# xultaeculcis/climate-super-resolution

Hardware: AMD Instinct MI355X
Metric: HR MPix/s per training step (4x SR, 64->256 tiles) (higher is better)
Workload: dtype bf16; 1 GPU; config 3: full ESRGAN GAN step (pl_gan.py:63-97: G pass = G fwd + D(hr), D(sr) + VGG19 perceptual + L1 + G bwd + AdamW_G; D pass = G fwd + D(hr), D(sr) + D bwd + AdamW_D; OneCycleLR x2); generator=ESRGAN nf64 nb11 gc16 x4, discriminator=RFBESRGANDiscriminator, global_batch=32, per_gpu_batch=32, lr_tile=64, hr_tile=256, parallelism=dp1, hip_graph=True, ddp_overlap=False, mode=gan

## Files before the change

### climate-super-resolution_amd/csrc/common.h

```cpp
#pragma once
#include <hip/hip_runtime.h>
#include <stdint.h>

#include "climsr_hip.h"

typedef __bf16 bf16x8 __attribute__((ext_vector_type(8)));
typedef __bf16 bf16x2 __attribute__((ext_vector_type(2)));
typedef short s16x4 __attribute__((ext_vector_type(4)));
typedef float f32x4 __attribute__((ext_vector_type(4)));

namespace climsr {

void set_error(const char* fmt, ...);
int check_launch(const char* what);
int device_cus();
int lds_opt_in(const void* fn, int bytes);

__device__ __forceinline__ uint16_t f2bf(float f) {
  __bf16 b = (__bf16)f;
  return __builtin_bit_cast(uint16_t, b);
}
__device__ __forceinline__ float bf2f(uint16_t u) { return __uint_as_float(((uint32_t)u) << 16); }

__device__ __forceinline__ float act_apply(float v, int act, float slope) {
// ... 15 lines not shown
constexpr uint32_t BUF_OOB = 0x80000000u;
__device__ __forceinline__ __amdgpu_buffer_rsrc_t buf_rsrc(const void* base, uint32_t bytes) {
  return __builtin_amdgcn_make_buffer_rsrc(const_cast<void*>(base), (short)0, (int)bytes, 0x00020000);
}
__device__ __forceinline__ uint4 buf_load16(__amdgpu_buffer_rsrc_t r, uint32_t off) {
  const auto v = __builtin_amdgcn_raw_buffer_load_b128(r, off, 0, 0);
  return make_uint4(v[0], v[1], v[2], v[3]);
}

__device__ __forceinline__ void lds_barrier() {
  __builtin_amdgcn_fence(__ATOMIC_RELEASE, "workgroup", "local");
  __builtin_amdgcn_s_barrier();
  __builtin_amdgcn_fence(__ATOMIC_ACQUIRE, "workgroup", "local");
}

static inline int ceil_div(long a, long b) { return (int)((a + b - 1) / b); }
static inline int round_up(int a, int b) { return (a + b - 1) / b * b; }

}
```

### climate-super-resolution_amd/csrc/conv.hip

```cpp
#include <atomic>
#include <mutex>
#include <stdarg.h>
#include <stdio.h>
#include <stdlib.h>

#include "common.h"
#include "conv_ep.h"
#include "conv_route.h"

namespace climsr {

static thread_local char g_err[512] = "";

void set_error(const char* fmt, ...) {
  va_list ap;
  va_start(ap, fmt);
  vsnprintf(g_err, sizeof(g_err), fmt, ap);
  va_end(ap);
}

int check_launch(const char* what) {
  hipError_t e = hipGetLastError();
  if (e != hipSuccess) {
    set_error("%s: %s", what, hipGetErrorString(e));
// ... 354 lines not shown
    r->geo = 2;
    if (r->pg.nvx <= 2 * 64 * r->nw) r->pv = 2;
  } else if (r->nw * r->mw == 16 && d->ks == 3 && d->cc == 64 && r->pg.kcpad == 9 * 64 && r->pg.ccp == 80 && r->pg.tpw == TW + 2 &&
             r->pg.tph == 18) {
    r->geo = 1;
  }
  r->tiles_y = ceil_div(d->out_h, r->nw * r->mw);
  return true;
}

static void pick_generic(const ClimsrConvDesc* d, bool bias, const ClimsrEpilogue* ep, bool bz, FwdRoute* r) {
  const FwdGeom& g = r->g;
  const bool r1 = ep->res1 != nullptr, r2 = ep->res2 != nullptr, aux = ep->aux != nullptr, bwd = ep->act == 3 || ep->act == 4;
  const bool al8 = (d->out_c & 7) == 0 && ((d->out_cstride | d->out_coff) & 7) == 0;
  const bool r1al8 = ((ep->res1_cstride | ep->res1_coff) & 7) == 0;
  const int plain = plain_ep(d, bias, ep);
  r->family = FAM_FWD; r->mw = g.mw; r->nt = g.nt;
  r->parts = bz && d->up == -2 && plain == 8 && dgrad_s2_shape(d, bias, ep);
  if (g.mw == 4) {
    const int nrx = ceil_div(g.tph * g.tpw * (d->cc / 8), 256), nrw = ceil_div(g.nt * 16 * (g.kcpad / 8), 256);
    r->nt = 4;
    if (g.nchunk > 1 && nrx <= 6 && nrw <= 9) {
      r->pfx = 6; r->pfw = 9;
      const bool v8 = al8 && r1al8 && (!r2 || ((ep->res2_cstride | ep->res2_coff) & 7) == 0) &&
                      (!aux || ((ep->aux_cstride | ep->aux_coff) & 7) == 0) && !ep->down2 && ep->act == 0 && r1;
      if (v8 && bias && ep->res_f32 == 0 && ep->out_mode == 0 && !aux) r->ep = 1;
      else if (v8 && !bias && (ep->res_f32 & 1) && (!r2 || (ep->res_f32 & 2)) && ep->out_mode == 1) r->ep = 2;
      else if (!bias && r1 && bwd && ep->res_f32 == 0 && !r2 && !aux && !ep->down2 && ep->out_mode == 0 && al8 && r1al8) r->ep = 4;
      else if (plain == 8) r->ep = bz ? 10 : ep->bn_part ? 9 : 8;
      else r->ep = plain;
      r->parts |= (r->ep == 9 || r->ep == 10) && d->out_c % 64 == 0 && d->out_c >= 128 && d->stride == 1 && d->up == 1 && d->ks == 3;
    } else if (g.nchunk > 1 && nrx <= 18 && nrw <= 9) {
      r->pfx = 18; r->pfw = 9; r->ep = plain == 8 ? 8 : 0;
    } else {
      r->ep = plain;
    }
    const bool base = d->cc == 32 && d->ks == 3 && g.kcpad == 9 * 32;
    if (r->pfx != 18 && base && d->stride == 1 && g.tpw == TW + 2 && g.ccp == 48 && d->up == 1 && d->in_c % 32 == 0 &&
        g.nchunk * 32 == d->in_c && (long)d->n * d->in_h * d->in_w * d->in_cstride * 2 < (1L << 31) &&
        (long)r->ncob * r->nt * 16 * g.kpk * 2 < (1L << 31))
      r->geo = 1;
    if (r->pfx == 18 && base && d->stride == 2 && g.tpw == 2 * TW + 1 && g.ccp == 40) r->geo = 2;
  }
  if (r->geo == 1) {
    const bool fits = (r->ep == 9 || r->ep == 10) ? d->out_h % DMA_TH == 0 : (d->out_h % DMA_TH == 0 || d->out_h >= 3 * DMA_TH);
    if (r->ep != 1 && r->ep != 2 && !ep->down2 && fits) {
      r->family = FAM_DMA;
      r->tiles_y = ceil_div(d->out_h, DMA_TH);
      r->xgrp = conv_xcd_group(r->ncob, (long)64 * g.kpk * 2);
      return;
    }
    r->xgrp = conv_xcd_group(r->ncob, (long)r->nt * 16 * g.kpk * 2);
  }
  const size_t lds_ep = (size_t)4 * r->mw * 16 * (r->nt * 16 + 4) * 4;
  r->lds = lds_ep > g.lds_total ? lds_ep : g.lds_total;
}

static int fwd_pick(const ClimsrConvDesc* d, bool bias, const ClimsrEpilogue* ep, FwdRoute* r) {
  *r = FwdRoute{};
  const bool cc4 = d->cc == 4 && d->in_c == 4;
  const bool bz = ep->bn_part && ep->bn_z, r1 = ep->res1 != nullptr, r2 = ep->res2 != nullptr, aux = ep->aux != nullptr;
// ... 52 lines not shown
}

static int fwd_route(const ClimsrConvDesc* d, bool bias, const ClimsrEpilogue* ep, FwdRoute* r) {
  if (!d || !ep) {
    set_error("conv2d_fwd: null argument");
    return CLIMSR_EINVAL;
  }
  const bool cc4 = d->cc == 4 && d->in_c == 4;
  if ((d->in_c % 8 && !cc4) || d->in_cstride % 8 || d->in_coff % 8 || (d->cc % 8 && !cc4) || d->cc <= 0 ||
      (d->up != 1 && d->up != 2 && d->up != -2) ||
      (d->stride != 1 && d->stride != 2) || d->ks < 1 || d->n <= 0 || d->out_c <= 0 || d->in_coff + d->in_c > d->in_cstride) {
    set_error("conv2d_fwd: unsupported geometry (in_c=%d cs=%d coff=%d cc=%d up=%d stride=%d ks=%d)", d->in_c, d->in_cstride,
              d->in_coff, d->cc, d->up, d->stride, d->ks);
    return CLIMSR_EINVAL;
  }
  if (ep->down2 && (ep->res2 || ep->res_f32 || bias || ep->act == 1 || ep->act == 2 || (ep->res1 && ep->act < 3) ||
                    (d->out_h & 1) || (d->out_w & 1))) {
    set_error("conv2d_fwd: down2 epilogue: no bias / forward activation / residual (act 3/4 mask only), even output size");
    return CLIMSR_EINVAL;
  }
  if (ep->act < 0 || ep->act > 4 || ((ep->act == 3 || ep->act == 4) && !ep->res1)) {
    set_error("conv2d_fwd: act %d invalid (3/4 need res1 = the activation output)", ep->act);
    return CLIMSR_EINVAL;
  }
  const int pick = fwd_pick(d, bias, ep, r);
  if (ep->ch_part && !(pick == PICK_OK && r->family == FAM_WR && (r->ep == 3 || r->ep == 4))) {
    set_error("conv2d_fwd: per-tile channel sums only from the 64 -> 64 3x3 register-resident conv "
              "(climsr_conv2d_fwd_ch_parts)");
    return CLIMSR_EINVAL;
  }
  if (ep->aux && ((ep->aux_cstride | ep->aux_coff) & 3)) {
    set_error("conv2d_fwd: aux channel stride/offset must be multiples of 4");
    return CLIMSR_EINVAL;
  }
  {
    const long opx = (long)d->n * d->out_h * d->out_w;
    const long r1b = ep->res1 ? opx * ep->res1_cstride * ((ep->res_f32 & 1) ? 4 : 2) : 0;
    const long r2b = ep->res2 ? opx * ep->res2_cstride * ((ep->res_f32 & 2) ? 4 : 2) : 0;
    const long yb = opx * d->out_cstride * (ep->out_mode == 0 ? 2 : 4);
    if (r1b >= (1L << 32) - 64 || r2b >= (1L << 32) - 64 || yb >= (1L << 32) - 64) {
      set_error("conv2d_fwd: output / residual operand of %ld B exceeds 32-bit buffer addressing (split the batch)",
// ... 130 lines not shown
```

### climate-super-resolution_amd/csrc/conv_dma.hip

```cpp
#include <algorithm>
#include <type_traits>

#include "conv_ep.h"

constexpr int DMA_TPW = TW + 2, DMA_XROW = DMA_TPW * 64;
constexpr int DMA_XU = (DMA_TH + 2) * DMA_TPW * 4;
constexpr int DMA_XI = (DMA_XU + 63) / 64;
constexpr int DMA_WI = 64 * 36 / 64;
constexpr int DMA_XB = DMA_XI * 1024, DMA_WB = DMA_WI * 1024, DMA_BUF = DMA_XB + DMA_WB;
constexpr int DMA_EPP = 64 + 4;
constexpr size_t DMA_LDS = std::max((size_t)2 * DMA_BUF, (size_t)8 * 64 * DMA_EPP * 4);
static_assert(DMA_LDS <= 160 * 1024, "LDS-DMA conv: two chunk buffers");


constexpr uint32_t ST_OOB = 0xFFFFFFC0u;
typedef unsigned int v4u32 __attribute__((ext_vector_type(4)));
template <int EP>
struct DmaEp {
  static constexpr bool F32 = EP == 2 || EP == 7;
  static constexpr int NSTORE = 4 * (F32 ? 2 : 1) + (EP == 2 ? 4 : 0);
};
template <int EP>
__device__ __forceinline__ void dma_store_half(const FwdArgs& a, const float* eb, int ehp, int lane, int nimg, int oyw, int ox0, int co0) {
  static_assert(EP == 1 || EP == 2 || EP == 3 || EP == 6 || EP == 7 || EP == 8, "persistent epilogues");
// ... 46 lines not shown
    if constexpr (EP == 2) __builtin_amdgcn_raw_buffer_store_b128(__builtin_bit_cast(v4u32, pack8_bf16(v, a.aux_scale)), rax, aoff[j], 0, 0);
  }
}

#ifndef CLIMSR_DMA_SPREAD
#define CLIMSR_DMA_SPREAD 1
#endif
#ifndef CLIMSR_DMA_DIAG
#define CLIMSR_DMA_DIAG 0
#endif

template <int EP, bool RF>
__global__ __launch_bounds__(512, 1) void conv_fwd_dma_kernel(FwdArgs a) {
  extern __shared__ __attribute__((aligned(16))) char smem[];
  constexpr bool BN = EP == 9 || EP == 10;
  constexpr bool CNT = EP == 1 || EP == 2 || EP == 3 || EP == 6 || EP == 7 || EP == 8;
  constexpr bool DIRECT = EP == 3 || EP == 6 || EP == 8;
  constexpr int NST_ITEM = DIRECT ? 16 : 2 * DmaEp<CNT ? EP : 8>::NSTORE;
  const int tid = threadIdx.x, wave = tid >> 6, lane = tid & 63, g = lane >> 4, col = lane & 15;
  const int wvu = __builtin_amdgcn_readfirstlane(wave);
  const int ntile = a.tiles_x * a.tiles_y * a.n, ncob = (a.out_c + 63) / 64;
  const int nitem = ntile * ncob;
  auto decode = [&](int v, int& nimg, int& oy0, int& ox0, int& co0, int& tyo) {
    int tile_id, cob;
    if (a.xgrp > 0) {
      const int idx = xcd_major(v, nitem), grp = idx / (ntile * a.xgrp), rem = idx - grp * (ntile * a.xgrp);
      tile_id = rem / a.xgrp;
      cob = grp * a.xgrp + (rem - tile_id * a.xgrp);
    } else {
      cob = v / ntile;
      tile_id = v - cob * ntile;
    }
    const int tx = tile_id % a.tiles_x, ty = (tile_id / a.tiles_x) % a.tiles_y;
// ... 137 lines not shown
      }
      lds_barrier();
      if ((wave & 3) == 0) {
        float ts = 0.f, tq = 0.f;
#pragma unroll
        for (int w = 0; w < 4; ++w) {
          ts += red[w * 128 + lane];
          tq += red[w * 128 + 64 + lane];
        }
        const long tile16 = ((long)nimg * (2 * a.tiles_y) + 2 * ty + (wave >> 2)) * a.tiles_x + ox0 / TW;
        double* out = a.bn_part + tile16 * 2 * a.out_c;
        out[co0 + lane] = (double)ts;
        out[a.out_c + co0 + lane] = (double)tq;
      }
      return;
    } else if (DIRECT) {
      const __amdgpu_buffer_rsrc_t ry = buf_rsrc(a.y, (uint32_t)((long)a.n * a.out_h * a.out_w * a.out_cs * 2));
      float bb[4][4];
#pragma unroll
      for (int t = 0; t < 4; ++t) {
        const float4 b4 = EP == 3 ? *(const float4*)(a.bias + co0 + 16 * t + 4 * g) : make_float4(0.f, 0.f, 0.f, 0.f);
        bb[t][0] = b4.x; bb[t][1] = b4.y; bb[t][2] = b4.z; bb[t][3] = b4.w;
      }
      const int ox = ox0 + col;
      uint32_t rowb[4];
#pragma unroll
      for (int m = 0; m < 4; ++m) {
        const int oy = oy0 + wave * 4 + m;
        const uint32_t pix = ((uint32_t)nimg * (uint32_t)a.out_h + (uint32_t)oy) * (uint32_t)a.out_w + (uint32_t)ox;
        rowb[m] = (oy < a.out_h && ox < a.out_w) ? (pix * (uint32_t)a.out_cs + (uint32_t)(a.out_co + co0 + 4 * g)) * 2u : BUF_OOB;
      }
// ... 37 lines not shown
    }
    if (vn >= nitem) break;
    v = vn;
    nimg = nimg_n; oy0 = oy0_n; ox0 = ox0_n; co0 = co0_n; ty = ty_n;
  }
}

namespace climsr {
int fwd_dma_launch(int ep, const FwdArgs& a, int ncob, hipStream_t s) {
  void (*k)(FwdArgs) = nullptr;
  const bool rf = a.res_f32 != 0;
#define DMA_EP(E) \
  case E: k = rf ? conv_fwd_dma_kernel<E, true> : conv_fwd_dma_kernel<E, false>; break;
  switch (ep) {
    DMA_EP(0) DMA_EP(3) DMA_EP(4) DMA_EP(6) DMA_EP(7) DMA_EP(8) DMA_EP(9) DMA_EP(10)
    default: set_error("conv2d_fwd: no LDS-DMA kernel for epilogue %d", ep); return CLIMSR_EINVAL;
  }
#undef DMA_EP
  if (int e = lds_opt_in((const void*)k, 160 * 1024)) return e;
  int ncu = device_cus();
  ncu = ncu >= 8 ? ncu / 8 * 8 : 8;
  const int nitem = a.tiles_x * a.tiles_y * a.n * ncob;
  const int grid = (ep == 9 || ep == 10) ? nitem : std::min(nitem, ncu);
  hipLaunchKernelGGL(k, dim3(grid), dim3(512), DMA_LDS, s, a);
  return CLIMSR_OK;
}
}

constexpr int S2D_TP = 33;
constexpr int S2D_XI = (S2D_TP * S2D_TP * 2 + 63) / 64;
// ... 202 lines not shown
```

### climate-super-resolution_amd/csrc/conv_wr.hip

```cpp
#include <algorithm>
#include <stdio.h>

#include "conv_route.h"
#include "mfma_agpr.h"

namespace {

constexpr int WR_TR = 4, WR_TC = 16;
constexpr int WR_PR = WR_TR + 2, WR_PC = WR_TC + 2;
constexpr int WR_XP = 80;
constexpr int WR_SPP = WR_XP / 8;
constexpr int WR_SLOTS = WR_PR * WR_PC * WR_SPP;
constexpr int WR_NI = (WR_SLOTS + 63) / 64;
constexpr int WR_BUF = WR_NI * 1024;
constexpr int WR_LDS = 4 * 2 * WR_BUF;
constexpr int WR_RED = 64 * 17 * 4;
constexpr int WR_LDS_ALL = WR_LDS + 4 * WR_RED;
static_assert(WR_LDS_ALL <= 160 * 1024, "conv_wr LDS");

struct WrArgs {
  const uint16_t* x;
  const uint16_t* w;
  const float* bias;
  uint16_t* y;
// ... 7 lines not shown
  uint32_t x_bytes, y_bytes, r1_bytes;
};
typedef uint32_t v2u32 __attribute__((ext_vector_type(2)));
typedef uint32_t v4u32 __attribute__((ext_vector_type(4)));

__device__ __forceinline__ float wr_axpby(bool fused, float x, float alpha, float beta, float r) {
#pragma clang fp contract(off)
  const float br = beta * r;
  if (fused) return __builtin_fmaf(x, alpha, br);
  const float xa = x * alpha;
  return xa + br;
}

template <int EP, int ACT>
__global__ __launch_bounds__(256, 1) void conv_wr_kernel(WrArgs a) {
  static_assert(EP == 2 ? (ACT == 3 || ACT == 4) : EP == 1 ? ACT == 0 : (ACT >= 0 && ACT <= 2), "conv_wr_ep()'s pairs");
  extern __shared__ __attribute__((aligned(16))) char smem[];
  constexpr int NEPI = EP == 0 ? 16 : (EP == 3 || EP == 4 ? 17 : 32);
  constexpr bool SUMS = EP == 3 || EP == 4;
  const int tid = threadIdx.x, lane = tid & 63, g = lane >> 4, col = lane & 15;
  const int wv = __builtin_amdgcn_readfirstlane(tid >> 6);
  const int G4 = (int)gridDim.x * 4;
  int T = xcd_major(blockIdx.x, gridDim.x) * 4 + wv;
  if (T >= a.ntiles) return;

  bf16x8 afb[4][18];
#pragma unroll
  for (int t = 0; t < 4; ++t)
#pragma unroll
    for (int j = 0; j < 18; ++j) afb[t][j] = *(const bf16x8*)(a.w + (long)(t * 16 + col) * a.kpk + j * 32 + g * 8);
  float bias[4][4];
#pragma unroll
  for (int t = 0; t < 4; ++t) {
// ... 79 lines not shown
#pragma unroll
    for (int j = 0; j < 18; ++j) {
      if (j + 1 < 18) ldb(j + 1, (j + 1) & 1);
      __builtin_amdgcn_sched_barrier(0);
#pragma unroll
      for (int m = 0; m < 4; ++m) {
        if (j == 0) mfma4x_agpr<true, false>(acc[m][0], acc[m][1], acc[m][2], acc[m][3], afb[0][j], afb[1][j], afb[2][j], afb[3][j], bq[0][m]);
        else if (j < 6) mfma4x_agpr<false, false>(acc[m][0], acc[m][1], acc[m][2], acc[m][3], afb[0][j], afb[1][j], afb[2][j], afb[3][j], bq[j & 1][m]);
        else mfma4x_agpr<false, true>(acc[m][0], acc[m][1], acc[m][2], acc[m][3], afb[0][j], afb[1][j], afb[2][j], afb[3][j], bq[j & 1][m]);
      }
      __builtin_amdgcn_sched_barrier(0);
    }
    pad_mfma16(acc);
    const int nimg = ni, oy0 = ty * WR_TR, ox0 = tx * WR_TC;
    const int ox = ox0 + col;
    uint32_t off[4];
    uint2 rv[4][4];
#pragma unroll
    for (int m = 0; m < 4; ++m) {
      const int oy = oy0 + m;
      const bool ok = oy < a.out_h && ox < a.out_w;
      const long pix = ((long)nimg * a.out_h + oy) * a.out_w + ox;
      off[m] = ok ? (uint32_t)((pix * a.out_cs + a.out_co + 4 * g) * (EP == 3 ? 4 : 2)) : BUF_OOB;
      if constexpr (EP == 1 || EP == 2) {
        const uint32_t ro = ok ? (uint32_t)((pix * a.r1_cs + a.r1_co + 4 * g) * 2) : BUF_OOB;
#pragma unroll
        for (int t = 0; t < 4; ++t) {
          const auto v = __builtin_amdgcn_raw_buffer_load_b64(rr, ro == BUF_OOB ? BUF_OOB : ro + (uint32_t)(t * 32), 0, 0);
          rv[m][t] = make_uint2(v[0], v[1]);
        }
      }
    }
    float csum[4][4] = {};
#pragma unroll
    for (int m = 0; m < 4; ++m)
#pragma unroll
      for (int t = 0; t < 4; ++t) {
        float v[4];
#pragma unroll
        for (int i = 0; i < 4; ++i) {
          float x = acc[m][t][i] + bias[t][i];
          if constexpr (EP == 2) {
            const uint32_t w = i < 2 ? rv[m][t].x : rv[m][t].y;
            const float r = __uint_as_float((i & 1) ? (w & 0xFFFF0000u) : (w << 16));
            x = r > 0.f ? x : (ACT == 3 ? x * a.slope : 0.f);
          } else {
            if constexpr (ACT == 1) x = x > 0.f ? x : x * a.slope;
            else if constexpr (ACT == 2) x = x > 0.f ? x : 0.f;
            if constexpr (EP == 1) {
              const uint32_t w = i < 2 ? rv[m][t].x : rv[m][t].y;
              const float r = __uint_as_float((i & 1) ? (w & 0xFFFF0000u) : (w << 16));
              x = wr_axpby(i < 3, x, a.alpha1, a.beta1, r);
            }
          }
          v[i] = x;
        }
        if constexpr (EP == 3) {
          const v4u32 pk = {__float_as_uint(v[0]), __float_as_uint(v[1]), __float_as_uint(v[2]), __float_as_uint(v[3])};
          __builtin_amdgcn_raw_buffer_store_b128(pk, yr, off[m] == BUF_OOB ? BUF_OOB : off[m] + (uint32_t)(t * 64), 0, 0);
          if (off[m] != BUF_OOB) {
#pragma unroll
            for (int i = 0; i < 4; ++i) csum[t][i] += v[i];
          }
        } else {
          const bf16x2 p0 = {(__bf16)v[0], (__bf16)v[1]}, p1 = {(__bf16)v[2], (__bf16)v[3]};
          const v2u32 pk = {__builtin_bit_cast(uint32_t, p0), __builtin_bit_cast(uint32_t, p1)};
          __builtin_amdgcn_raw_buffer_store_b64(pk, yr, off[m] == BUF_OOB ? BUF_OOB : off[m] + (uint32_t)(t * 32), 0, 0);
          if (EP == 4 && off[m] != BUF_OOB) {
#pragma unroll
            for (int i = 0; i < 4; ++i) csum[t][i] += v[i];
          }
        }
      }
    if constexpr (SUMS) {
      float* red = (float*)(smem + WR_LDS) + wv * (WR_RED / 4);
#pragma unroll
      for (int t = 0; t < 4; ++t)
#pragma unroll
        for (int i = 0; i < 4; ++i) red[(16 * t + 4 * g + i) * 17 + col] = csum[t][i];
      float cs = 0.f;
#pragma unroll
      for (int c = 0; c < 16; ++c) cs += red[lane * 17 + c];
      __builtin_amdgcn_raw_buffer_store_b32(__float_as_uint(cs), pr, (uint32_t)((T * 64 + lane) * 4), 0, 0);
    }
    if (Tn >= a.ntiles) break;
    T = Tn;
    tx = txn; ty = tyn; ni = nin;
  }
  asm volatile("s_waitcnt vmcnt(0)" ::: "memory");
}

}

namespace climsr {

int conv_wr_ep(const ClimsrConvDesc* d, const ClimsrEpilogue* ep, bool bias) {
  const bool res = ep->res1 != nullptr;
  int epk = -1;
  if (ep->out_mode == 0 && !res && ep->act >= 0 && ep->act <= 2) epk = ep->ch_part ? 4 : 0;
  else if (ep->out_mode == 0 && res && ep->act == 0 && !(ep->res_f32 & 1)) epk = 1;
  else if (ep->out_mode == 0 && res && (ep->act == 3 || ep->act == 4) && !bias && !(ep->res_f32 & 1)) epk = 2;
  else if (ep->out_mode == 1 && !res && ep->act >= 0 && ep->act <= 2) epk = 3;
  const long opx = (long)d->n * d->out_h * d->out_w;
  if (epk < 0 || (ep->ch_part && epk != 3 && epk != 4) || d->in_c != 64 || d->out_c != 64 || d->cc != 64 || d->ks != 3 || d->stride != 1 ||
      d->pad != 1 || (d->up != 1 && d->up != 2) || d->out_h != d->in_h * d->up || d->out_w != d->in_w * d->up ||
      d->in_cstride % 8 || d->in_coff % 8 || (d->out_cstride | d->out_coff) & 3 || ep->down2 || ep->res2 || ep->aux ||
      ep->bn_part || (res && ((ep->res1_cstride | ep->res1_coff) & 3)) ||
      (long)d->n * d->in_h * d->in_w * d->in_cstride * 2 >= (1L << 31) ||
      opx * d->out_cstride * (epk == 3 ? 4 : 2) >= (1L << 31) || (res && opx * ep->res1_cstride * 2 >= (1L << 31)) ||
      (long)ceil_div(d->out_w, WR_TC) * ceil_div(d->out_h, WR_TR) * d->n * 256 >= (1L << 31))
    return -1;
  return epk;
}

int conv_wr_tiles_per_image(const ClimsrConvDesc* d) { return ceil_div(d->out_w, WR_TC) * ceil_div(d->out_h, WR_TR); }

int conv_wr_launch(int epk, const ClimsrConvDesc* d, const ClimsrEpilogue* ep, const uint16_t* x, const uint16_t* wpk, int kpk,
                   const float* bias, void* y, hipStream_t s) {
  const bool res = ep->res1 != nullptr;
  const long opx = (long)d->n * d->out_h * d->out_w;
  WrArgs a;
  a.x = x; a.w = wpk; a.bias = bias; a.y = (uint16_t*)y; a.res1 = (const uint16_t*)ep->res1; a.ch_part = ep->ch_part;
  a.n = d->n; a.in_h = d->in_h; a.in_w = d->in_w; a.in_cs = d->in_cstride; a.in_co = d->in_coff; a.up = d->up;
  a.out_h = d->out_h; a.out_w = d->out_w; a.out_cs = d->out_cstride; a.out_co = d->out_coff; a.kpk = kpk;
  a.act = ep->act; a.slope = ep->slope; a.alpha1 = ep->alpha1; a.beta1 = ep->beta1;
  a.r1_cs = ep->res1_cstride; a.r1_co = ep->res1_coff;
  a.tiles_x = ceil_div(d->out_w, WR_TC); a.tiles_y = ceil_div(d->out_h, WR_TR);
  a.ntiles = a.tiles_x * a.tiles_y * d->n;
  a.x_bytes = (uint32_t)((long)d->n * d->in_h * d->in_w * d->in_cstride * 2);
  a.y_bytes = (uint32_t)(opx * d->out_cstride * (epk == 3 ? 4 : 2));
  a.r1_bytes = res ? (uint32_t)(opx * ep->res1_cstride * 2) : 0u;
  const int ncu = device_cus();
  const int grid = std::min(ceil_div(a.ntiles, 4), ncu);
  void (*k)(WrArgs) = nullptr;
#define WR_ACT3(E) (a.act == 1 ? conv_wr_kernel<E, 1> : a.act == 2 ? conv_wr_kernel<E, 2> : conv_wr_kernel<E, 0>)
  switch (epk) {
    case 0: k = WR_ACT3(0); break;
    case 1: k = conv_wr_kernel<1, 0>; break;
    case 2: k = a.act == 3 ? conv_wr_kernel<2, 3> : conv_wr_kernel<2, 4>; break;
    case 3: k = WR_ACT3(3); break;
    default: k = WR_ACT3(4); break;
  }
#undef WR_ACT3
  const int lds = (epk == 3 || epk == 4) ? WR_LDS_ALL : WR_LDS;
  if (int e = lds_opt_in((const void*)k, WR_LDS_ALL)) return e;
  hipLaunchKernelGGL(k, dim3(grid), dim3(256), lds, s, a);
  return check_launch("conv2d_fwd (wr)");
}

}
```

### climate-super-resolution_amd/losses/perceptual.py

```python
from typing import List

import numpy as np
import torch
import torch.nn as nn

from .. import ops
from ..core.init import init_state, spec_from_shapes
from ..ops import ACT_NONE, ACT_RELU, ConvPlan, OUT_BF16

VGG19_E = [64, 64, "M", 128, 128, "M", 256, 256, 256, 256, "M", 512, 512, 512, 512, "M", 512, 512, 512, 512, "M"]


def _vgg19_features_35() -> nn.Sequential:
    layers: List[nn.Module] = []
    cin = 3
    for v in VGG19_E:
        if v == "M":
            layers.append(nn.MaxPool2d(kernel_size=2, stride=2))
        else:
            layers += [nn.Conv2d(cin, v, kernel_size=3, padding=1), nn.ReLU(inplace=True)]
            cin = v
    return nn.Sequential(*layers[:35])


class PerceptualLoss(nn.Module):

    def __init__(self, deterministic_init: bool = True):
        super().__init__()
        loss_network = _vgg19_features_35().eval()
        if deterministic_init:
            shapes = {k: tuple(v.shape) for k, v in loss_network.state_dict().items()}
            st = init_state(spec_from_shapes({"loss_network." + k: s for k, s in shapes.items()}), gain=float(np.sqrt(6.0)))
            loss_network.load_state_dict({k[len("loss_network."):]: torch.from_numpy(np.asarray(v)) for k, v in st.items()})
        for param in loss_network.parameters():
            param.requires_grad = False
        self.loss_network = loss_network
        self._plans = None
        self._dev = None

    def _build(self, dev):
        plans = []
        mods = list(self.loss_network)
        for i, m in enumerate(mods):
            if isinstance(m, nn.Conv2d):
                relu = i + 1 < len(mods) and isinstance(mods[i + 1], nn.ReLU)
                pool = i + 2 < len(mods) and isinstance(mods[i + 2], nn.MaxPool2d)
                p = ConvPlan(m.in_channels, m.out_channels, 3, 1, 1, f"loss_network.{i}")
                w = m.weight.detach().contiguous().float()
                b = m.bias.detach().contiguous().float()
                p.bind(w, b, need_t=False)
                p.pack()
                plans.append((p, relu, pool))
        self._plans = plans
        self._dev = dev
        self._version = sum(int(p.weight._version) for p, _r, _q in plans)

    def features(self, x3: torch.Tensor, n: int, h: int, w: int) -> torch.Tensor:
        a, cs = x3, 8
        for p, relu, pool in self._plans:
            y = torch.empty((n, h, w, p.cout), dtype=torch.bfloat16, device=x3.device)
            p.fwd(a, cs, 0, h, w, y, p.cout, 0, n, act=ACT_RELU if relu else ACT_NONE, out_mode=OUT_BF16)
            a, cs = y, p.cout
            if pool:
                h2, w2 = h // 2, w // 2
                yp = torch.empty((n, h2, w2, cs), dtype=torch.bfloat16, device=x3.device)
                ops.maxpool2(a, n, h, w, cs, yp)
                a, h, w = yp, h2, w2
        return a

    @torch.no_grad()
    def forward(self, fake_high_resolution, high_resolution):
        a, b = fake_high_resolution, high_resolution
        if not a.is_cuda:
            raise RuntimeError("climsr_amd.PerceptualLoss runs on the GPU only (no CPU fallback)")
# ... 15 lines not shown
```

### climate-super-resolution_amd/ops.py

```python
from __future__ import annotations

import ctypes
import os
from typing import Optional

import torch

from . import _lib
from ._lib import ChainDesc, ConvDesc, Epilogue, PackDesc, PullPackDesc, ReduceDesc, check, ptr

ACT_NONE, ACT_LRELU, ACT_RELU = 0, 1, 2
ACT_LRELU_BWD, ACT_RELU_BWD = 3, 4
OUT_BF16, OUT_F32, OUT_F32_ADD = 0, 1, 2


def round_up(a: int, b: int) -> int:
    return (a + b - 1) // b * b


PROFILER = None


def _kname(d, bias, ep) -> str:
    if PROFILER is None:
# ... 72 lines not shown
            out.append(PackDesc(ptr(self.weight), ptr(self.wpk_t), self.cout_t, self.cin_t, self.cout, self.cout_t, self.ks,
                                self.cc_t, 1, 0))
        return out

    def out_hw(self, in_h: int, in_w: int, up: int = 1):
        h = (in_h * up + 2 * self.pad - self.ks) // self.stride + 1
        w = (in_w * up + 2 * self.pad - self.ks) // self.stride + 1
        return h, w

    def fwd(self, x: torch.Tensor, x_cs: int, x_co: int, in_h: int, in_w: int, y: torch.Tensor, y_cs: int, y_co: int,
            n: int, up: int = 1, act: int = ACT_NONE, slope: float = 0.2, use_bias: bool = True,
            res1: Optional[torch.Tensor] = None, alpha1: float = 1.0, res1_cs: int = 0, res1_co: int = 0,
            res2: Optional[torch.Tensor] = None, alpha2: float = 1.0, res2_cs: int = 0, res2_co: int = 0,
            out_mode: int = OUT_BF16, beta1: float = 1.0, beta2: float = 1.0, aux: Optional[torch.Tensor] = None,
            aux_cs: int = 0, aux_co: int = 0, aux_scale: float = 1.0, bn_part: Optional[torch.Tensor] = None,
            ch_part: Optional[torch.Tensor] = None) -> None:
        oh, ow = self.out_hw(in_h, in_w, up)
        if (self.cin_real == 1 and self.ks in (3, 5) and self.stride == 1 and self.pad == self.ks // 2 and up == 1
                and self.cout in (32, 64) and out_mode == OUT_BF16 and y.dtype == torch.bfloat16 and res1 is None and res2 is None
                and aux is None and act in (ACT_NONE, ACT_LRELU, ACT_RELU) and (y_cs | y_co) % 8 == 0):
            px = n * oh * ow
            b = ptr(self.bias) if (use_bias and self.bias is not None) else None
            kn = "dgrad_ci1_kernel<%d, %d, true>" % (self.ks, self.cout // 8) if PROFILER is not None else ""
            _run(kn, 2 * self.cout * self.ks * self.ks * px, lambda: check(
                _lib.load().climsr_conv_single_input(n, in_h, in_w, self.ks, self.pad, ptr(x), x_cs, x_co, ptr(self.weight), b,
                                                     self.cout, act, slope, ptr(y), y_cs, y_co, _lib.stream_ptr()),
                f"conv fwd {self.name}"), "fwd " + self.name, px * 2 + px * self.cout * 2)
            return
        d = ConvDesc(n, in_h, in_w, self.cin_k, x_cs, x_co, up, self.ks, self.stride, self.pad, oh, ow, self.cout, y_cs, y_co,
                     self.cc)
        rf = (1 if res1 is not None and res1.dtype == torch.float32 else 0) | \
             (2 if res2 is not None and res2.dtype == torch.float32 else 0)
        ep = Epilogue(act, slope, alpha1, ptr(res1), res1_cs, res1_co, alpha2, ptr(res2), res2_cs, res2_co, out_mode, 0,
                      rf, beta1, beta2, aux_cs, ptr(aux), aux_co, aux_scale, ptr(bn_part), ch_part=ptr(ch_part))
        b = ptr(self.bias) if (use_bias and self.bias is not None) else None
        flops = 2 * self.cin_real * self.cout * self.ks * self.ks * n * oh * ow
        opx = n * oh * ow
        nbytes = (n * in_h * in_w * self.cin_real * 2 + self.rows * self.kpk * 2 +
                  opx * self.cout * (y.element_size() * (2 if out_mode == OUT_F32_ADD else 1) + _esize(res1) + _esize(res2) +
                                     _esize(aux)))
        _run(_kname(d, b, ep), flops, lambda: check(
            _lib.load().climsr_conv2d_fwd(ctypes.byref(d), ptr(x), ptr(self.wpk), b, ctypes.byref(ep), ptr(y), _lib.stream_ptr()),
            f"conv fwd {self.name}"), "fwd " + self.name, nbytes)

    def bn_parts(self, x_cs: int, in_h: int, in_w: int, n: int, y_cs: int) -> int:
        oh, ow = self.out_hw(in_h, in_w)
        d = ConvDesc(n, in_h, in_w, self.cin_k, x_cs, 0, 1, self.ks, self.stride, self.pad, oh, ow, self.cout, y_cs, 0, self.cc)
        ep = Epilogue(ACT_NONE, 0.0, 1.0, None, 0, 0, 1.0, None, 0, 0, OUT_BF16, 0, 0, 1.0, 1.0, 0, None, 0, 1.0, 1)
        return int(_lib.load().climsr_conv2d_fwd_bn_parts(ctypes.byref(d), ctypes.byref(ep)))

    def ch_parts(self, x_cs: int, in_h: int, in_w: int, n: int, y_cs: int) -> tuple:
        oh, ow = self.out_hw(in_h, in_w)
        d = ConvDesc(n, in_h, in_w, self.cin_k, x_cs, 0, 1, self.ks, self.stride, self.pad, oh, ow, self.cout, y_cs, 0, self.cc)
        ep = Epilogue(ACT_NONE, 0.0, 1.0, None, 0, 0, 1.0, None, 0, 0, OUT_F32, 0, 0, 1.0, 1.0, 0, None, 0, 1.0, None)
        tpi = ctypes.c_int32(0)
        rows = int(_lib.load().climsr_conv2d_fwd_ch_parts(ctypes.byref(d), ctypes.byref(ep), ctypes.byref(tpi)))
        return rows, int(tpi.value)

# ... 470 lines not shown
```

Measured before the change: 85.77 HR MPix/s.

## Fuse 2x2 max-pool into VGG conv epilogues for perceptual loss

Adds a max-pool epilogue mode (down2 = 2) to the register-resident 64->64 conv and the LDS-DMA conv. Each 2x2 window is reduced in registers with a DPP lane swap, then bias and ReLU are applied and only the pooled bf16 map is stored. The VGG19 perceptual-loss forward uses this for conv+ReLU+pool layers, which removes the full-resolution activation write and the separate pool kernel read. It adds new epilogue variants and routing checks. Layers that don't qualify fall back to the existing conv plus pool path.

```diff
diff --git a/climate-super-resolution_amd/csrc/common.h b/climate-super-resolution_amd/csrc/common.h
--- a/climate-super-resolution_amd/csrc/common.h
+++ b/climate-super-resolution_amd/csrc/common.h
@@ -53,6 +53,10 @@
   __builtin_amdgcn_fence(__ATOMIC_ACQUIRE, "workgroup", "local");
 }
 
+__device__ __forceinline__ float quad_swap1(float x) {
+  return __builtin_bit_cast(float, __builtin_amdgcn_update_dpp(0, __builtin_bit_cast(int, x), 0xB1, 0xF, 0xF, true));
+}
+
 static inline int ceil_div(long a, long b) { return (int)((a + b - 1) / b); }
 static inline int round_up(int a, int b) { return (a + b - 1) / b * b; }
 
diff --git a/climate-super-resolution_amd/csrc/conv.hip b/climate-super-resolution_amd/csrc/conv.hip
--- a/climate-super-resolution_amd/csrc/conv.hip
+++ b/climate-super-resolution_amd/csrc/conv.hip
@@ -392,7 +392,10 @@
   const bool r1 = ep->res1 != nullptr, r2 = ep->res2 != nullptr, aux = ep->aux != nullptr, bwd = ep->act == 3 || ep->act == 4;
   const bool al8 = (d->out_c & 7) == 0 && ((d->out_cstride | d->out_coff) & 7) == 0;
   const bool r1al8 = ((ep->res1_cstride | ep->res1_coff) & 7) == 0;
-  const int plain = plain_ep(d, bias, ep);
+  const bool pool = ep->down2 == 2;
+  ClimsrEpilogue unpooled = *ep;
+  unpooled.down2 = 0;
+  const int plain = plain_ep(d, bias, pool ? &unpooled : ep);
   r->family = FAM_FWD; r->mw = g.mw; r->nt = g.nt;
   r->parts = bz && d->up == -2 && plain == 8 && dgrad_s2_shape(d, bias, ep);
   if (g.mw == 4) {
@@ -422,7 +425,9 @@
   }
   if (r->geo == 1) {
     const bool fits = (r->ep == 9 || r->ep == 10) ? d->out_h % DMA_TH == 0 : (d->out_h % DMA_TH == 0 || d->out_h >= 3 * DMA_TH);
-    if (r->ep != 1 && r->ep != 2 && !ep->down2 && fits) {
+    const bool pooled = pool && r->ep == 3 && ep->act == 2 && d->out_c % 64 == 0;
+    if (r->ep != 1 && r->ep != 2 && (!ep->down2 || pooled) && fits) {
+      if (pooled) r->ep = 11;
       r->family = FAM_DMA;
       r->tiles_y = ceil_div(d->out_h, DMA_TH);
       r->xgrp = conv_xcd_group(r->ncob, (long)64 * g.kpk * 2);
@@ -505,7 +510,26 @@
               d->in_coff, d->cc, d->up, d->stride, d->ks);
     return CLIMSR_EINVAL;
   }
-  if (ep->down2 && (ep->res2 || ep->res_f32 || bias || ep->act == 1 || ep->act == 2 || (ep->res1 && ep->act < 3) ||
+  if (ep->down2 == 2) {
+    if (ep->act != 2 || !bias) {
+      set_error("conv2d_fwd: max-pool epilogue (down2 = 2) needs a bias and ReLU (act 2), got act %d%s", ep->act, bias ? "" : ", no bias");
+      return CLIMSR_EINVAL;
+    }
+    if (ep->out_mode != 0) {
+      set_error("conv2d_fwd: max-pool epilogue (down2 = 2) stores bf16 only (out_mode %d)", ep->out_mode);
+      return CLIMSR_EINVAL;
+    }
+    if (ep->res1 || ep->res2 || ep->res_f32 || ep->aux || ep->bn_part || ep->ch_part) {
+      set_error("conv2d_fwd: max-pool epilogue (down2 = 2) takes no residual, aux output, BatchNorm partials or channel sums");
+      return CLIMSR_EINVAL;
+    }
+    if ((d->out_h & 1) || (d->out_w & 1) || d->up != 1 || d->stride != 1) {
+      set_error("conv2d_fwd: max-pool epilogue (down2 = 2) needs an even output size (%d x %d), up 1 and stride 1 (up %d, stride %d)",
+                d->out_h, d->out_w, d->up, d->stride);
+      return CLIMSR_EINVAL;
+    }
+  }
+  if (ep->down2 && ep->down2 != 2 && (ep->res2 || ep->res_f32 || bias || ep->act == 1 || ep->act == 2 || (ep->res1 && ep->act < 3) ||
                     (d->out_h & 1) || (d->out_w & 1))) {
     set_error("conv2d_fwd: down2 epilogue: no bias / forward activation / residual (act 3/4 mask only), even output size");
     return CLIMSR_EINVAL;
@@ -515,7 +539,12 @@
     return CLIMSR_EINVAL;
   }
   const int pick = fwd_pick(d, bias, ep, r);
-  if (ep->ch_part && !(pick == PICK_OK && r->family == FAM_WR && (r->ep == 3 || r->ep == 4))) {
+  if (ep->down2 == 2 && !(pick == PICK_OK && ((r->family == FAM_WR && r->ep == 5) || (r->family == FAM_DMA && r->ep == 11)))) {
+    set_error("conv2d_fwd: max-pool epilogue (down2 = 2) only from the 64 -> 64 register-resident conv and the LDS-DMA conv "
+              "(climsr_conv2d_fwd_kernel names the kernel, or nothing); run the conv and climsr_maxpool2_bf16 instead");
+    return CLIMSR_EINVAL;
+  }
+  if (ep->ch_part &&!(pick == PICK_OK && r->family == FAM_WR && (r->ep == 3 || r->ep == 4))) {
     set_error("conv2d_fwd: per-tile channel sums only from the 64 -> 64 3x3 register-resident conv "
               "(climsr_conv2d_fwd_ch_parts)");
     return CLIMSR_EINVAL;
diff --git a/climate-super-resolution_amd/csrc/conv_dma.hip b/climate-super-resolution_amd/csrc/conv_dma.hip
--- a/climate-super-resolution_amd/csrc/conv_dma.hip
+++ b/climate-super-resolution_amd/csrc/conv_dma.hip
@@ -84,9 +84,10 @@
 __global__ __launch_bounds__(512, 1) void conv_fwd_dma_kernel(FwdArgs a) {
   extern __shared__ __attribute__((aligned(16))) char smem[];
   constexpr bool BN = EP == 9 || EP == 10;
-  constexpr bool CNT = EP == 1 || EP == 2 || EP == 3 || EP == 6 || EP == 7 || EP == 8;
-  constexpr bool DIRECT = EP == 3 || EP == 6 || EP == 8;
-  constexpr int NST_ITEM = DIRECT ? 16 : 2 * DmaEp<CNT ? EP : 8>::NSTORE;
+  constexpr bool CNT = EP == 1 || EP == 2 || EP == 3 || EP == 6 || EP == 7 || EP == 8 || EP == 11;
+  constexpr bool POOL = EP == 11;
+  constexpr bool DIRECT = EP == 3 || EP == 6 || EP == 8 || POOL;
+  constexpr int NST_ITEM = POOL ? 4 : DIRECT ? 16 : 2 * DmaEp<CNT ? EP : 8>::NSTORE;
   const int tid = threadIdx.x, wave = tid >> 6, lane = tid & 63, g = lane >> 4, col = lane & 15;
   const int wvu = __builtin_amdgcn_readfirstlane(wave);
   const int ntile = a.tiles_x * a.tiles_y * a.n, ncob = (a.out_c + 63) / 64;
@@ -254,7 +255,29 @@
         out[a.out_c + co0 + lane] = (double)tq;
       }
       return;
-    } else if (DIRECT) {
+    } else if constexpr (POOL) {
+      const __amdgpu_buffer_rsrc_t ry = buf_rsrc(a.y, (uint32_t)((long)a.n * (a.out_h >> 1) * (a.out_w >> 1) * a.out_cs * 2));
+      const int odd = col & 1, oy = oy0 + wave * 4 + 2 * odd, ox = ox0 + col;
+      const uint32_t pix = ((uint32_t)nimg * (uint32_t)(a.out_h >> 1) + (uint32_t)(oy >> 1)) * (uint32_t)(a.out_w >> 1) + (uint32_t)(ox >> 1);
+      const uint32_t pb = (oy < a.out_h && ox < a.out_w) ? (pix * (uint32_t)a.out_cs + (uint32_t)(a.out_co + co0 + 4 * g)) * 2u : BUF_OOB;
+      float4 bb[4];
+#pragma unroll
+      for (int t = 0; t < 4; ++t) bb[t] = *(const float4*)(a.bias + co0 + 16 * t + 4 * g);
+#pragma unroll
+      for (int t = 0; t < 4; ++t) {
+        const float bt[4] = {bb[t].x, bb[t].y, bb[t].z, bb[t].w};
+        float v[4];
+#pragma unroll
+        for (int i = 0; i < 4; ++i) {
+          const float r01 = fmaxf(acc[0][t][i], acc[1][t][i]), r23 = fmaxf(acc[2][t][i], acc[3][t][i]);
+          v[i] = act_apply(fmaxf(odd ? r23 : r01, quad_swap1(odd ? r01 : r23)) + bt[i], 2, 0.f);
+        }
+        const bf16x2 p0 = {(__bf16)v[0], (__bf16)v[1]}, p1 = {(__bf16)v[2], (__bf16)v[3]};
+        typedef uint32_t v2u32_t __attribute__((ext_vector_type(2)));
+        const v2u32_t pk = {__builtin_bit_cast(uint32_t, p0), __builtin_bit_cast(uint32_t, p1)};
+        __builtin_amdgcn_raw_buffer_store_b64(pk, ry, pb == BUF_OOB ? BUF_OOB : pb + (uint32_t)(32 * t), 0, 0);
+      }
+    } else if constexpr (DIRECT) {
       const __amdgpu_buffer_rsrc_t ry = buf_rsrc(a.y, (uint32_t)((long)a.n * a.out_h * a.out_w * a.out_cs * 2));
       float bb[4][4];
 #pragma unroll
@@ -322,6 +345,7 @@
   case E: k = rf ? conv_fwd_dma_kernel<E, true> : conv_fwd_dma_kernel<E, false>; break;
   switch (ep) {
     DMA_EP(0) DMA_EP(3) DMA_EP(4) DMA_EP(6) DMA_EP(7) DMA_EP(8) DMA_EP(9) DMA_EP(10)
+    case 11: k = conv_fwd_dma_kernel<11, false>; break;
     default: set_error("conv2d_fwd: no LDS-DMA kernel for epilogue %d", ep); return CLIMSR_EINVAL;
   }
 #undef DMA_EP
diff --git a/climate-super-resolution_amd/csrc/conv_wr.hip b/climate-super-resolution_amd/csrc/conv_wr.hip
--- a/climate-super-resolution_amd/csrc/conv_wr.hip
+++ b/climate-super-resolution_amd/csrc/conv_wr.hip
@@ -45,9 +45,10 @@
 
 template <int EP, int ACT>
 __global__ __launch_bounds__(256, 1) void conv_wr_kernel(WrArgs a) {
-  static_assert(EP == 2 ? (ACT == 3 || ACT == 4) : EP == 1 ? ACT == 0 : (ACT >= 0 && ACT <= 2), "conv_wr_ep()'s pairs");
+  static_assert(EP == 2 ? (ACT == 3 || ACT == 4) : EP == 1 ? ACT == 0 : EP == 5 ? ACT == 2 : (ACT >= 0 && ACT <= 2),
+                "conv_wr_ep()'s pairs");
   extern __shared__ __attribute__((aligned(16))) char smem[];
-  constexpr int NEPI = EP == 0 ? 16 : (EP == 3 || EP == 4 ? 17 : 32);
+  constexpr int NEPI = EP == 0 ? 16 : EP == 5 ? 4 : (EP == 3 || EP == 4 ? 17 : 32);
   constexpr bool SUMS = EP == 3 || EP == 4;
   const int tid = threadIdx.x, lane = tid & 63, g = lane >> 4, col = lane & 15;
   const int wv = __builtin_amdgcn_readfirstlane(tid >> 6);
@@ -157,74 +158,94 @@
     pad_mfma16(acc);
     const int nimg = ni, oy0 = ty * WR_TR, ox0 = tx * WR_TC;
     const int ox = ox0 + col;
-    uint32_t off[4];
-    uint2 rv[4][4];
-#pragma unroll
-    for (int m = 0; m < 4; ++m) {
-      const int oy = oy0 + m;
-      const bool ok = oy < a.out_h && ox < a.out_w;
-      const long pix = ((long)nimg * a.out_h + oy) * a.out_w + ox;
-      off[m] = ok ? (uint32_t)((pix * a.out_cs + a.out_co + 4 * g) * (EP == 3 ? 4 : 2)) : BUF_OOB;
-      if constexpr (EP == 1 || EP == 2) {
-        const uint32_t ro = ok ? (uint32_t)((pix * a.r1_cs + a.r1_co + 4 * g) * 2) : BUF_OOB;
-#pragma unroll
-        for (int t = 0; t < 4; ++t) {
-          const auto v = __builtin_amdgcn_raw_buffer_load_b64(rr, ro == BUF_OOB ? BUF_OOB : ro + (uint32_t)(t * 32), 0, 0);
-          rv[m][t] = make_uint2(v[0], v[1]);
-        }
-      }
-    }
-    float csum[4][4] = {};
-#pragma unroll
-    for (int m = 0; m < 4; ++m)
+    if constexpr (EP == 5) {
+      const int odd = col & 1;
+      const bool ok = oy0 + 2 * odd < a.out_h && ox < a.out_w;
+      const long pix = ((long)nimg * (a.out_h >> 1) + (oy0 >> 1) + odd) * (a.out_w >> 1) + (ox >> 1);
+      const uint32_t po = ok ? (uint32_t)((pix * a.out_cs + a.out_co + 4 * g) * 2) : BUF_OOB;
 #pragma unroll
       for (int t = 0; t < 4; ++t) {
         float v[4];
 #pragma unroll
         for (int i = 0; i < 4; ++i) {
-          float x = acc[m][t][i] + bias[t][i];
-          if constexpr (EP == 2) {
-            const uint32_t w = i < 2 ? rv[m][t].x : rv[m][t].y;
-            const float r = __uint_as_float((i & 1) ? (w & 0xFFFF0000u) : (w << 16));
-            x = r > 0.f ? x : (ACT == 3 ? x * a.slope : 0.f);
-          } else {
-            if constexpr (ACT == 1) x = x > 0.f ? x : x * a.slope;
-            else if constexpr (ACT == 2) x = x > 0.f ? x : 0.f;
-            if constexpr (EP == 1) {
+          const float r01 = fmaxf(acc[0][t][i], acc[1][t][i]), r23 = fmaxf(acc[2][t][i], acc[3][t][i]);
+          const float x = fmaxf(odd ? r23 : r01, quad_swap1(odd ? r01 : r23)) + bias[t][i];
+          v[i] = x > 0.f ? x : 0.f;
+        }
+        const bf16x2 p0 = {(__bf16)v[0], (__bf16)v[1]}, p1 = {(__bf16)v[2], (__bf16)v[3]};
+        const v2u32 pk = {__builtin_bit_cast(uint32_t, p0), __builtin_bit_cast(uint32_t, p1)};
+        __builtin_amdgcn_raw_buffer_store_b64(pk, yr, po == BUF_OOB ? BUF_OOB : po + (uint32_t)(t * 32), 0, 0);
+      }
+    } else {
+      uint32_t off[4];
+      uint2 rv[4][4];
+#pragma unroll
+      for (int m = 0; m < 4; ++m) {
+        const int oy = oy0 + m;
+        const bool ok = oy < a.out_h && ox < a.out_w;
+        const long pix = ((long)nimg * a.out_h + oy) * a.out_w + ox;
+        off[m] = ok ? (uint32_t)((pix * a.out_cs + a.out_co + 4 * g) * (EP == 3 ? 4 : 2)) : BUF_OOB;
+        if constexpr (EP == 1 || EP == 2) {
+          const uint32_t ro = ok ? (uint32_t)((pix * a.r1_cs + a.r1_co + 4 * g) * 2) : BUF_OOB;
+#pragma unroll
+          for (int t = 0; t < 4; ++t) {
+            const auto v = __builtin_amdgcn_raw_buffer_load_b64(rr, ro == BUF_OOB ? BUF_OOB : ro + (uint32_t)(t * 32), 0, 0);
+            rv[m][t] = make_uint2(v[0], v[1]);
+          }
+        }
+      }
+      float csum[4][4] = {};
+#pragma unroll
+      for (int m = 0; m < 4; ++m)
+#pragma unroll
+        for (int t = 0; t < 4; ++t) {
+          float v[4];
+#pragma unroll
+          for (int i = 0; i < 4; ++i) {
+            float x = acc[m][t][i] + bias[t][i];
+            if constexpr (EP == 2) {
               const uint32_t w = i < 2 ? rv[m][t].x : rv[m][t].y;
               const float r = __uint_as_float((i & 1) ? (w & 0xFFFF0000u) : (w << 16));
-              x = wr_axpby(i < 3, x, a.alpha1, a.beta1, r);
+              x = r > 0.f ? x : (ACT == 3 ? x * a.slope : 0.f);
+            } else {
+              if constexpr (ACT == 1) x = x > 0.f ? x : x * a.slope;
+              else if constexpr (ACT == 2) x = x > 0.f ? x : 0.f;
+              if constexpr (EP == 1) {
+                const uint32_t w = i < 2 ? rv[m][t].x : rv[m][t].y;
+                const float r = __uint_as_float((i & 1) ? (w & 0xFFFF0000u) : (w << 16));
+                x = wr_axpby(i < 3, x, a.alpha1, a.beta1, r);
+              }
+            }
+            v[i] = x;
+          }
+          if constexpr (EP == 3) {
+            const v4u32 pk = {__float_as_uint(v[0]), __float_as_uint(v[1]), __float_as_uint(v[2]), __float_as_uint(v[3])};
+            __builtin_amdgcn_raw_buffer_store_b128(pk, yr, off[m] == BUF_OOB ? BUF_OOB : off[m] + (uint32_t)(t * 64), 0, 0);
+            if (off[m] != BUF_OOB) {
+#pragma unroll
+              for (int i = 0; i < 4; ++i) csum[t][i] += v[i];
+            }
+          } else {
+            const bf16x2 p0 = {(__bf16)v[0], (__bf16)v[1]}, p1 = {(__bf16)v[2], (__bf16)v[3]};
+            const v2u32 pk = {__builtin_bit_cast(uint32_t, p0), __builtin_bit_cast(uint32_t, p1)};
+            __builtin_amdgcn_raw_buffer_store_b64(pk, yr, off[m] == BUF_OOB ? BUF_OOB : off[m] + (uint32_t)(t * 32), 0, 0);
+            if (EP == 4 && off[m] != BUF_OOB) {
+#pragma unroll
+              for (int i = 0; i < 4; ++i) csum[t][i] += v[i];
             }
           }
-          v[i] = x;
         }
-        if constexpr (EP == 3) {
-          const v4u32 pk = {__float_as_uint(v[0]), __float_as_uint(v[1]), __float_as_uint(v[2]), __float_as_uint(v[3])};
-          __builtin_amdgcn_raw_buffer_store_b128(pk, yr, off[m] == BUF_OOB ? BUF_OOB : off[m] + (uint32_t)(t * 64), 0, 0);
-          if (off[m] != BUF_OOB) {
-#pragma unroll
-            for (int i = 0; i < 4; ++i) csum[t][i] += v[i];
-          }
-        } else {
-          const bf16x2 p0 = {(__bf16)v[0], (__bf16)v[1]}, p1 = {(__bf16)v[2], (__bf16)v[3]};
-          const v2u32 pk = {__builtin_bit_cast(uint32_t, p0), __builtin_bit_cast(uint32_t, p1)};
-          __builtin_amdgcn_raw_buffer_store_b64(pk, yr, off[m] == BUF_OOB ? BUF_OOB : off[m] + (uint32_t)(t * 32), 0, 0);
-          if (EP == 4 && off[m] != BUF_OOB) {
-#pragma unroll
-            for (int i = 0; i < 4; ++i) csum[t][i] += v[i];
-          }
-        }
-      }
-    if constexpr (SUMS) {
-      float* red = (float*)(smem + WR_LDS) + wv * (WR_RED / 4);
-#pragma unroll
-      for (int t = 0; t < 4; ++t)
-#pragma unroll
-        for (int i = 0; i < 4; ++i) red[(16 * t + 4 * g + i) * 17 + col] = csum[t][i];
-      float cs = 0.f;
-#pragma unroll
-      for (int c = 0; c < 16; ++c) cs += red[lane * 17 + c];
-      __builtin_amdgcn_raw_buffer_store_b32(__float_as_uint(cs), pr, (uint32_t)((T * 64 + lane) * 4), 0, 0);
+      if constexpr (SUMS) {
+        float* red = (float*)(smem + WR_LDS) + wv * (WR_RED / 4);
+#pragma unroll
+        for (int t = 0; t < 4; ++t)
+#pragma unroll
+          for (int i = 0; i < 4; ++i) red[(16 * t + 4 * g + i) * 17 + col] = csum[t][i];
+        float cs = 0.f;
+#pragma unroll
+        for (int c = 0; c < 16; ++c) cs += red[lane * 17 + c];
+        __builtin_amdgcn_raw_buffer_store_b32(__float_as_uint(cs), pr, (uint32_t)((T * 64 + lane) * 4), 0, 0);
+      }
     }
     if (Tn >= a.ntiles) break;
     T = Tn;
@@ -240,14 +261,17 @@
 int conv_wr_ep(const ClimsrConvDesc* d, const ClimsrEpilogue* ep, bool bias) {
   const bool res = ep->res1 != nullptr;
   int epk = -1;
-  if (ep->out_mode == 0 && !res && ep->act >= 0 && ep->act <= 2) epk = ep->ch_part ? 4 : 0;
+  if (ep->down2 == 2) {
+    const bool even = !((d->out_h | d->out_w) & 1);
+    epk = (ep->out_mode == 0 && !res && ep->act == 2 && bias && !ep->ch_part && d->up == 1 && even) ? 5 : -1;
+  } else if (ep->out_mode == 0 && !res && ep->act >= 0 && ep->act <= 2) epk = ep->ch_part ? 4 : 0;
   else if (ep->out_mode == 0 && res && ep->act == 0 && !(ep->res_f32 & 1)) epk = 1;
   else if (ep->out_mode == 0 && res && (ep->act == 3 || ep->act == 4) && !bias && !(ep->res_f32 & 1)) epk = 2;
   else if (ep->out_mode == 1 && !res && ep->act >= 0 && ep->act <= 2) epk = 3;
   const long opx = (long)d->n * d->out_h * d->out_w;
   if (epk < 0 || (ep->ch_part && epk != 3 && epk != 4) || d->in_c != 64 || d->out_c != 64 || d->cc != 64 || d->ks != 3 || d->stride != 1 ||
       d->pad != 1 || (d->up != 1 && d->up != 2) || d->out_h != d->in_h * d->up || d->out_w != d->in_w * d->up ||
-      d->in_cstride % 8 || d->in_coff % 8 || (d->out_cstride | d->out_coff) & 3 || ep->down2 || ep->res2 || ep->aux ||
+      d->in_cstride % 8 || d->in_coff % 8 || (d->out_cstride | d->out_coff) & 3 || (ep->down2 && epk != 5) || ep->res2 || ep->aux ||
       ep->bn_part || (res && ((ep->res1_cstride | ep->res1_coff) & 3)) ||
       (long)d->n * d->in_h * d->in_w * d->in_cstride * 2 >= (1L << 31) ||
       opx * d->out_cstride * (epk == 3 ? 4 : 2) >= (1L << 31) || (res && opx * ep->res1_cstride * 2 >= (1L << 31)) ||
@@ -271,7 +295,7 @@
   a.tiles_x = ceil_div(d->out_w, WR_TC); a.tiles_y = ceil_div(d->out_h, WR_TR);
   a.ntiles = a.tiles_x * a.tiles_y * d->n;
   a.x_bytes = (uint32_t)((long)d->n * d->in_h * d->in_w * d->in_cstride * 2);
-  a.y_bytes = (uint32_t)(opx * d->out_cstride * (epk == 3 ? 4 : 2));
+  a.y_bytes = (uint32_t)((epk == 5 ? opx / 4 : opx) * d->out_cstride * (epk == 3 ? 4 : 2));
   a.r1_bytes = res ? (uint32_t)(opx * ep->res1_cstride * 2) : 0u;
   const int ncu = device_cus();
   const int grid = std::min(ceil_div(a.ntiles, 4), ncu);
@@ -282,6 +306,7 @@
     case 1: k = conv_wr_kernel<1, 0>; break;
     case 2: k = a.act == 3 ? conv_wr_kernel<2, 3> : conv_wr_kernel<2, 4>; break;
     case 3: k = WR_ACT3(3); break;
+    case 5: k = conv_wr_kernel<5, 2>; break;
     default: k = WR_ACT3(4); break;
   }
 #undef WR_ACT3
diff --git a/climate-super-resolution_amd/losses/perceptual.py b/climate-super-resolution_amd/losses/perceptual.py
--- a/climate-super-resolution_amd/losses/perceptual.py
+++ b/climate-super-resolution_amd/losses/perceptual.py
@@ -25,8 +25,9 @@
 
 class PerceptualLoss(nn.Module):
 
-    def __init__(self, deterministic_init: bool = True):
+    def __init__(self, deterministic_init: bool = True, fuse_pool: bool = True):
         super().__init__()
+        self.fuse_pool = fuse_pool
         loss_network = _vgg19_features_35().eval()
         if deterministic_init:
             shapes = {k: tuple(v.shape) for k, v in loss_network.state_dict().items()}
@@ -37,6 +38,7 @@
         self.loss_network = loss_network
         self._plans = None
         self._dev = None
+        self._fused = {}
 
     def _build(self, dev):
         plans = []
@@ -53,11 +55,31 @@
                 plans.append((p, relu, pool))
         self._plans = plans
         self._dev = dev
+        self._fused = {}
         self._version = sum(int(p.weight._version) for p, _r, _q in plans)
+
+    def _pool_fused(self, n: int, h: int, w: int):
+        key = (n, h, w)
+        if key not in self._fused:
+            out, cs = [], 8
+            for p, relu, pool in self._plans:
+                ok = self.fuse_pool and relu and pool and h % 2 == 0 and w % 2 == 0 and p.pool2_ok(cs, 0, h, w, n, p.cout)
+                out.append(ok)
+                cs = p.cout
+                if pool:
+                    h, w = h // 2, w // 2
+            self._fused[key] = out
+        return self._fused[key]
 
     def features(self, x3: torch.Tensor, n: int, h: int, w: int) -> torch.Tensor:
         a, cs = x3, 8
-        for p, relu, pool in self._plans:
+        for (p, relu, pool), fused in zip(self._plans, self._pool_fused(n, h, w)):
+            if fused:
+                h2, w2 = h // 2, w // 2
+                yp = torch.empty((n, h2, w2, p.cout), dtype=torch.bfloat16, device=x3.device)
+                p.fwd(a, cs, 0, h, w, yp, p.cout, 0, n, act=ACT_RELU, out_mode=OUT_BF16, pool2=True)
+                a, cs, h, w = yp, p.cout, h2, w2
+                continue
             y = torch.empty((n, h, w, p.cout), dtype=torch.bfloat16, device=x3.device)
             p.fwd(a, cs, 0, h, w, y, p.cout, 0, n, act=ACT_RELU if relu else ACT_NONE, out_mode=OUT_BF16)
             a, cs = y, p.cout
diff --git a/climate-super-resolution_amd/ops.py b/climate-super-resolution_amd/ops.py
--- a/climate-super-resolution_amd/ops.py
+++ b/climate-super-resolution_amd/ops.py
@@ -110,9 +110,9 @@
             res2: Optional[torch.Tensor] = None, alpha2: float = 1.0, res2_cs: int = 0, res2_co: int = 0,
             out_mode: int = OUT_BF16, beta1: float = 1.0, beta2: float = 1.0, aux: Optional[torch.Tensor] = None,
             aux_cs: int = 0, aux_co: int = 0, aux_scale: float = 1.0, bn_part: Optional[torch.Tensor] = None,
-            ch_part: Optional[torch.Tensor] = None) -> None:
+            ch_part: Optional[torch.Tensor] = None, pool2: bool = False) -> None:
         oh, ow = self.out_hw(in_h, in_w, up)
-        if (self.cin_real == 1 and self.ks in (3, 5) and self.stride == 1 and self.pad == self.ks // 2 and up == 1
+        if (self.cin_real == 1 and self.ks in (3, 5) and self.stride == 1 and self.pad == self.ks // 2 and up == 1 and not pool2
                 and self.cout in (32, 64) and out_mode == OUT_BF16 and y.dtype == torch.bfloat16 and res1 is None and res2 is None
                 and aux is None and act in (ACT_NONE, ACT_LRELU, ACT_RELU) and (y_cs | y_co) % 8 == 0):
             px = n * oh * ow
@@ -127,17 +127,26 @@
                      self.cc)
         rf = (1 if res1 is not None and res1.dtype == torch.float32 else 0) | \
              (2 if res2 is not None and res2.dtype == torch.float32 else 0)
-        ep = Epilogue(act, slope, alpha1, ptr(res1), res1_cs, res1_co, alpha2, ptr(res2), res2_cs, res2_co, out_mode, 0,
-                      rf, beta1, beta2, aux_cs, ptr(aux), aux_co, aux_scale, ptr(bn_part), ch_part=ptr(ch_part))
+        ep = Epilogue(act, slope, alpha1, ptr(res1), res1_cs, res1_co, alpha2, ptr(res2), res2_cs, res2_co, out_mode,
+                      2 if pool2 else 0, rf, beta1, beta2, aux_cs, ptr(aux), aux_co, aux_scale, ptr(bn_part), ch_part=ptr(ch_part))
         b = ptr(self.bias) if (use_bias and self.bias is not None) else None
         flops = 2 * self.cin_real * self.cout * self.ks * self.ks * n * oh * ow
-        opx = n * oh * ow
+        opx = n * oh * ow // (4 if pool2 else 1)
         nbytes = (n * in_h * in_w * self.cin_real * 2 + self.rows * self.kpk * 2 +
                   opx * self.cout * (y.element_size() * (2 if out_mode == OUT_F32_ADD else 1) + _esize(res1) + _esize(res2) +
                                      _esize(aux)))
         _run(_kname(d, b, ep), flops, lambda: check(
             _lib.load().climsr_conv2d_fwd(ctypes.byref(d), ptr(x), ptr(self.wpk), b, ctypes.byref(ep), ptr(y), _lib.stream_ptr()),
             f"conv fwd {self.name}"), "fwd " + self.name, nbytes)
+
+    def pool2_ok(self, x_cs: int, x_co: int, in_h: int, in_w: int, n: int, y_cs: int, y_co: int = 0, act: int = ACT_RELU,
+                 use_bias: bool = True, out_mode: int = OUT_BF16) -> bool:
+        oh, ow = self.out_hw(in_h, in_w)
+        d = ConvDesc(n, in_h, in_w, self.cin_k, x_cs, x_co, 1, self.ks, self.stride, self.pad, oh, ow, self.cout, y_cs, y_co,
+                     self.cc)
+        ep = Epilogue(act, 0.0, 1.0, None, 0, 0, 1.0, None, 0, 0, out_mode, 2, 0, 1.0, 1.0, 0, None, 0, 1.0, None)
+        b = 1 if (use_bias and self.bias is not None) else None
+        return bool(_lib.load().climsr_conv2d_fwd_kernel(ctypes.byref(d), b, ctypes.byref(ep)))
 
     def bn_parts(self, x_cs: int, in_h: int, in_w: int, n: int, y_cs: int) -> int:
         oh, ow = self.out_hw(in_h, in_w)
```

Measured after the change: 87.11 HR MPix/s (median of 6 runs). +1.6%, better.
